# PranjalSahu/tensorflow_distributed

Hardware: AMD Instinct MI355X
Metric: images/sec (whole node) MNIST CNN DP at 1/2/4/8 MI355X; step-time scaling (higher is better)
Workload: dtype bf16; 1 GPU; global_batch=128, per_gpu_batch=128, parallelism=dp1, grad_allreduce=bf16, hipgraph=True, steps_per_graph=20, dp_transport=none, force_dp=False, zero1_fc1=False, fc_grads=bf16

## Files before the change

csrc/kernels/mnist.hip:

```cpp
#include "../common.h"

#include "../gemm.h"
#include "../gemm256.h"
#include "../launch_check.h"
#include "../mnist_layout.h"
#include "../tfd_kernels.h"
#include "../wt_store.h"
#include "../mnist_tail.h"

#include <algorithm>
#include <stdexcept>

constexpr int GEMM_RS = 2;
constexpr int FDX_BK_ = 128;
constexpr int FDW_BK_ = 64;
constexpr int FC1_BK_ = 32;

namespace tfd {
using namespace mnist;

namespace {

__device__ __forceinline__ int data_row(const int* perm, const int64_t* step, int n_data, int B, int b) {
  if (!perm) return b;
  const int64_t s = *step;
  return perm[(int)((s * (int64_t)B + b) % (int64_t)n_data)];
}
__device__ __forceinline__ int data_row(const MnistStepArgs& a, int b) {
  if (!a.perm) return b;
  if (a.rows) {
    const int tag = a.rows[a.B], r = a.rows[b];
    const int64_t s = *a.step;
    if (tag == (int)s) return r;
    return a.perm[(int)((s * (int64_t)a.B + b) % (int64_t)a.n_data)];
  }
  return data_row(a.perm, a.step, a.n_data, a.B, b);
}
struct RowPre {
  int64_t step;
  int tag, row;
};
__device__ __forceinline__ RowPre data_row_pre(const MnistStepArgs& a, int b) {
  RowPre r{0, -1, b};
  if (a.perm) {
    r.step = *a.step;
    if (a.rows) { r.tag = a.rows[a.B]; r.row = a.rows[b]; }
  }
  return r;
}
__device__ __forceinline__ int data_row_use(const MnistStepArgs& a, const RowPre& r, int b) {
  if (!a.perm) return b;
  if (a.rows && r.tag == (int)r.step) return r.row;
  return a.perm[(int)((r.step * (int64_t)a.B + b) % (int64_t)a.n_data)];
}
__device__ __forceinline__ int batch_label(const MnistStepArgs& a, int b) {
  if (a.perm && a.xpre) {
    const int tag = a.rows[a.B], y = a.ypre[b];
    const int64_t s = *a.step;
    if (tag == (int)s) return y;
  }
  return a.labels[data_row(a, b)];
}


constexpr int C2F_W = 24, C2F_PLANE = 18 * C2F_W, C2F_WLD = 48;
__device__ __forceinline__ int c2f_wrow(int r) { return (r >> 3) * 384 + (r & 7) * 32 + ((r >> 3) & 1) * 16; }
constexpr int C2F_WTAP = 4 * 384;
constexpr int C2F_WR4 = 4 * 32;
static_assert(C2F_WTAP == 32 * C2F_WLD, "the layout keeps the [800][48] footprint");
constexpr int C2L_FWD_SMEM = (4 * C2F_PLANE * 8 + 800 * C2F_WLD) * 2;
__device__ __forceinline__ void conv2_taps(const bf16* img, const bf16* wcol, const int base[2], f32x4 acc[2][2]) {
  bf16x8 a[2][2], b[2][2];
  auto load = [&](int tap, int slot) {
    const int kh = tap / 5, kw = tap - 5 * kh, toff = (kh * C2F_W + kw) * 8;
    const bf16* wr = wcol + tap * C2F_WTAP;
    b[slot][0] = frag_tr16(wr, wr + C2F_WR4);
    b[slot][1] = frag_tr16(wr + 16, wr + 16 + C2F_WR4);
    a[slot][0] = *reinterpret_cast<const bf16x8*>(img + base[0] + toff);
    a[slot][1] = *reinterpret_cast<const bf16x8*>(img + base[1] + toff);
  };
  load(0, 0);
#pragma unroll
  for (int tap = 0; tap < 25; ++tap) {
    const int cur = tap & 1;
    if (tap + 1 < 25) load(tap + 1, cur ^ 1);
#pragma unroll
    for (int j = 0; j < 2; ++j) {
      acc[j][0] = mfma16x16x32(a[cur][j], b[cur][0], acc[j][0]);
      acc[j][1] = mfma16x16x32(a[cur][j], b[cur][1], acc[j][1]);
    }
  }
}
static_assert(C2F_PLANE * 16 % 256 == 0, "chunk planes must be bank-row aligned");

constexpr int C12_XS = 36;
constexpr int C12_XR = 60;
constexpr int C12_XOFF = C2L_FWD_SMEM;
constexpr int C12_WOFF = C12_XOFF + C12_XR * C12_XS * 4;
constexpr int C12_IOFF = C12_WOFF + (KTAPS * C1 + C1) * 4;
constexpr int C12_X8P = 40;
constexpr int C12_X8OFF = C12_IOFF + 196 * 32;
constexpr int C12_SMEM = C12_X8OFF + 32 * C12_X8P * 16;
static_assert(C12_X8OFF % 16 == 0 && C12_SMEM <= 160 * 1024, "conv12 LDS carve");
static_assert(C12_IOFF % 16 == 0, "LDS carve alignment");
#ifndef TFD_STAMP
#define TFD_STAMP 0
#endif
#define C12_STAMP(k)                                                                       \
  do {                                                                                     \
    if (TFD_STAMP && a.dbg && threadIdx.x == 0) a.dbg[blockIdx.x * 16 + (k)] = (int64_t)__builtin_amdgcn_s_memtime(); \
  } while (0)
#define C12_STAMPW(k)                                                                      \
  do {                                                                                     \
    if (TFD_STAMP && a.dbg && threadIdx.x == 256) a.dbg[blockIdx.x * 16 + 8 + (k)] = (int64_t)__builtin_amdgcn_s_memtime(); \
  } while (0)
__global__ __launch_bounds__(512) void conv12_fwd_lds(MnistStepArgs a) {
  C12_STAMP(0);
  C12_STAMPW(0);
  extern __shared__ __attribute__((aligned(16))) char smem_raw[];
  bf16* img = (bf16*)smem_raw;
  bf16* wt = img + 4 * C2F_PLANE * 8;
  float* xs = reinterpret_cast<float*>(smem_raw + C12_XOFF);
  float* w1 = reinterpret_cast<float*>(smem_raw + C12_WOFF);
  const int b = blockIdx.x >> 1, nh = blockIdx.x & 1, t = threadIdx.x;
  const uint16_t* wsrc = a.pbf + OFF_WC2 + nh * 32;
  const int rot = (int)((blockIdx.x * 1031u) % 3200u);
  constexpr int NW = (3200 + 255) / 256;
  uint4 vw[NW];
#pragma unroll
  for (int j = 0; j < NW; ++j) vw[j] = zero4();
  f32x4 xv = f32x4{0.f, 0.f, 0.f, 0.f}, w1v = f32x4{0.f, 0.f, 0.f, 0.f};
  const int u = t - 256;
  const bool w2_role = __builtin_amdgcn_readfirstlane(t >> 6) < 4;
  if (w2_role) {
    const int tw = t & 255;
#pragma unroll
    for (int j = 0; j < NW; ++j) {
      const int e = tw + 256 * j, i = (min(e, 3199) + rot) % 3200;
      vw[j] = *reinterpret_cast<const uint4*>(wsrc + (i >> 2) * 64 + (i & 3) * 8);
    }
  } else {
    const int uw = min(u, (KTAPS * C1 + C1) / 4 - 1), ux = min(u, 195);
    w1v = reinterpret_cast<const f32x4*>(a.p32 + OFF_WC1)[uw];
    bool hit = false;
    if (a.perm && a.xpre) {
      xv = reinterpret_cast<const f32x4*>(a.xpre + (size_t)b * 784)[ux];
      hit = a.rows[a.B] == (int)*a.step;
    }
    if (!hit) {
      const float* x = a.data + (size_t)data_row(a, b) * 784;
      xv = reinterpret_cast<const f32x4*>(x)[ux];
    }
  }
  C12_STAMP(1);
  C12_STAMPW(1);
#if TFD_STAMP
  if (t == 256) {
    __builtin_amdgcn_s_waitcnt(0);
    C12_STAMPW(2);
  }
#endif
  for (int i = t; i < C12_XR * C12_XS / 4; i += 512) reinterpret_cast<f32x4*>(xs)[i] = f32x4{0.f, 0.f, 0.f, 0.f};
  for (int i = t; i < 4 * C2F_PLANE; i += 512) reinterpret_cast<uint4*>(img)[i] = zero4();
  C12_STAMPW(3);
  __syncthreads();
  C12_STAMPW(4);
  if (t >= 256) {
    if (u < (KTAPS * C1 + C1) / 4) reinterpret_cast<f32x4*>(w1)[u] = w1v;
    if (u < 196) {
      const int r = (4 * u) / 28, c = (4 * u) % 28;
      float* d = xs + (r + 2) * C12_XS + c + 2;
      d[0] = xv[0]; d[1] = xv[1]; d[2] = xv[2]; d[3] = xv[3];
    }
  }
  C12_STAMPW(5);
  __syncthreads();
  {
    bf16* x8 = reinterpret_cast<bf16*>(smem_raw + C12_X8OFF);
    for (int i = t; i < 32 * 28; i += 512) {
      const int r = i / 28, c = i - r * 28;
      const float* src = xs + r * C12_XS + c;
      bf16x8 e;
#pragma unroll
      for (int j = 0; j < 8; ++j) e[j] = (bf16)(j < 5 ? src[j] : 0.f);
      *reinterpret_cast<bf16x8*>(x8 + (r * C12_X8P + c) * 8) = e;
    }
    __syncthreads();
  }
  C12_STAMP(2);
  C12_STAMPW(6);
  {
    const int lane = t & 63, w = t >> 6, g = lane >> 4, col = lane & 15;
    uint8_t* idx_l = reinterpret_cast<uint8_t*>(smem_raw + C12_IOFF);
    const float bias0 = w1[KTAPS * C1 + col], bias1 = w1[KTAPS * C1 + 16 + col];
    constexpr int MT = 7;
    bf16x8 bw1[2], bw2[2];
#pragma unroll
    for (int nt = 0; nt < 2; ++nt)
#pragma unroll
      for (int jj = 0; jj < 8; ++jj) {
        const float r4 = jj < 5 ? w1[(20 + jj) * C1 + nt * 16 + col] : 0.f;
        bw1[nt][jj] = (bf16)(jj < 5 ? w1[(g * 5 + jj) * C1 + nt * 16 + col] : 0.f);
        bw2[nt][jj] = (bf16)(g == 0 ? r4 : 0.f);
      }
    const bf16* x8 = reinterpret_cast<const bf16*>(smem_raw + C12_X8OFF);
    bf16x8 af[MT], af2[MT];
#pragma unroll
    for (int i = 0; i < MT; ++i) {
      const int mt = w + 8 * i;
      const int m = min(mt, 48) * 16 + col, pp = m >> 2, win = m & 3;
      const int orow = 2 * (pp / 14) + (win >> 1), ocol = 2 * (pp % 14) + (win & 1);
      af[i] = *reinterpret_cast<const bf16x8*>(x8 + ((orow + g) * C12_X8P + ocol) * 8);
      af2[i] = *reinterpret_cast<const bf16x8*>(x8 + ((orow + 4) * C12_X8P + ocol) * 8);
    }
    f32x4 z[MT][2];
#pragma unroll
    for (int i = 0; i < MT; ++i)
#pragma unroll
      for (int nt = 0; nt < 2; ++nt)
        z[i][nt] = mfma16x16x32(af2[i], bw2[nt], mfma16x16x32(af[i], bw1[nt], f32x4{0.f, 0.f, 0.f, 0.f}));
#pragma unroll
    for (int i = 0; i < MT; ++i) {
      const int mt = w + 8 * i;
      if (mt >= 49) break;
      const int pq = mt * 4 + g, ph = pq / 14, pw = pq - ph * 14;
#pragma unroll
      for (int nt = 0; nt < 2; ++nt) {
        const int n = nt * 16 + col;
        const float bias = nt ? bias1 : bias0;
        float mx = z[i][nt][0] + bias;
        int am = 0;
#pragma unroll
        for (int r = 1; r < 4; ++r) {
          const float zz = z[i][nt][r] + bias;
          if (zz > mx) { mx = zz; am = r; }
        }
        reinterpret_cast<uint16_t*>(img)[((n >> 3) * C2F_PLANE + (ph + 2) * C2F_W + pw + 2) * 8 + (n & 7)] =
            f2bf_bits(fmaxf(mx, 0.f));
        idx_l[pq * 32 + n] = (uint8_t)am;
      }
    }
  }
  C12_STAMP(3);
  if (w2_role) {
#pragma unroll
    for (int j = 0; j < NW; ++j) {
      const int i = (t + 256 * j + rot) % 3200;
      if (t + 256 * j < 3200) *reinterpret_cast<uint4*>(wt + c2f_wrow(i >> 2) + (i & 3) * 8) = vw[j];
    }
  }
  __syncthreads();
  if (nh == 0) {
    const uint8_t* idx_l = reinterpret_cast<const uint8_t*>(smem_raw + C12_IOFF);
    const WtBuf bp1 = wt_buf(a.p1 + (size_t)b * 196 * 32, 196 * 32 * 2), bi1 = wt_buf(a.idx1 + (size_t)b * 196 * 32, 196 * 32);
    for (int i = t; i < 196 * 4; i += 512) {
      const int pq = i >> 2, cg = i & 3, ph = pq / 14, pw = pq - ph * 14;
      wt_store16(bp1, (uint32_t)i * 16u, true,
                 *reinterpret_cast<const uint4*>(img + (cg * C2F_PLANE + (ph + 2) * C2F_W + pw + 2) * 8));
    }
    for (int i = t; i < 196 * 2; i += 512) wt_store16(bi1, (uint32_t)i * 16u, true, reinterpret_cast<const uint4*>(idx_l)[i]);
  }
  C12_STAMP(4);
  const int lane = t & 63, w = t >> 6, g = lane >> 4, q = (lane & 15) >> 2, p4 = lane & 3;
  const int nmt = (w + 8 < 13) ? 2 : 1;
  int base[2];
  f32x4 acc[2][2];
#pragma unroll
  for (int j = 0; j < 2; ++j) {
    acc[j][0] = acc[j][1] = f32x4{0.f, 0.f, 0.f, 0.f};
    const int m = (w + 8 * j) * 16 + (lane & 15);
    int px = 0;
    if (m < 196) {
      const int pp = m >> 2, win = m & 3;
      px = (2 * (pp / 7) + (win >> 1)) * C2F_W + 2 * (pp % 7) + (win & 1);
    }
    base[j] = (g * C2F_PLANE + px) * 8;
  }
  const bf16* wcol = wt + c2f_wrow(8 * g + q) + 4 * p4;
  float bbv[2];
#pragma unroll
  for (int nt = 0; nt < 2; ++nt) bbv[nt] = a.p32[OFF_BC2 + nh * 32 + nt * 16 + (lane & 15)];
  conv2_taps(img, wcol, base, acc);
  C12_STAMP(5);
#pragma unroll
  for (int nt = 0; nt < 2; ++nt) {
    const int n = nh * 32 + nt * 16 + (lane & 15);
    const float bb = bbv[nt];
#pragma unroll
    for (int j = 0; j < 2; ++j) {
      const int m4 = (w + 8 * j) * 16 + 4 * g;
      if (j >= nmt || m4 >= 196) continue;
      float mx = acc[j][nt][0] + bb;
      int am = 0;
#pragma unroll
      for (int r = 1; r < 4; ++r) {
        const float z = acc[j][nt][r] + bb;
        if (z > mx) { mx = z; am = r; }
      }
      const size_t o = (size_t)b * FEAT + (m4 >> 2) * 64 + n;
      a.p2[o] = f2bf_bits(fmaxf(mx, 0.f));
      a.idx2[o] = (uint8_t)am;
    }
  }
  C12_STAMP(6);
}

struct SlabEpi {
  float* __restrict__ out;
  int ld, M, N;
  __device__ __forceinline__ void operator()(int m4, int n, f32x4 v) const {
    if (n >= N) return;
#pragma unroll
    for (int r = 0; r < 4; ++r)
      if (m4 + r < M) out[(size_t)(m4 + r) * ld + n] = v[r];
  }
};
constexpr int FC1_BM = 64, FC1_BN = 64, FC1_BK = FC1_BK_;
constexpr int FC1_SPLITS = 7;
constexpr int FC1_NKT = FEAT / FC1_SPLITS / FC1_BK;
static_assert(FC1_NKT * FC1_BK * FC1_SPLITS == FEAT, "fc1 split-K must tile K exactly");
__global__ __launch_bounds__(256) void fc1_fwd(MnistStepArgs a, int kper) {
  extern __shared__ __attribute__((aligned(16))) char smem_raw[];
  static_assert(FEAT % 8 == 0 && HID % 8 == 0, "whole chunks (DenseLoaderX)");
  DenseLoaderX<true> la{a.p2, FEAT, a.B, FEAT};
  DenseLoaderX<false> lb{a.pbf + OFF_WD1, HID, HID, FEAT};
  const int z = blockIdx.z;
  SlabEpi epi{a.fc1_slab + (size_t)z * a.B * HID, HID, a.B, HID};
  const int kb = z * kper;
  gemm_block_oneshot<FC1_BM, FC1_BN, FC1_BK, FC1_NKT, 2, 2>(la, lb, epi, blockIdx.y * FC1_BM, blockIdx.x * FC1_BN, kb, (bf16*)smem_raw);
}

#define HEAD_STAMP(k)                                                                                    \
  do {                                                                                                   \
    if (TFD_STAMP && a.dbg && threadIdx.x == 0) a.dbg[4 * a.B * 8 + blockIdx.x * 8 + (k)] = (int64_t)__builtin_amdgcn_s_memtime(); \
  } while (0)
__global__ __launch_bounds__(256) void head_kernel(MnistStepArgs a, int train) {
  HEAD_STAMP(0);
  const int row = blockIdx.x, t = threadIdx.x, lane = t & 63, wv = t >> 6;
  const int n0 = 4 * t;
  f32x4 p[FC1_SPLITS];
#pragma unroll
  for (int s = 0; s < FC1_SPLITS; ++s) p[s] = *reinterpret_cast<const f32x4*>(a.fc1_slab + ((size_t)s * a.B + row) * HID + n0);
  f32x4 wo[NCLS];
#pragma unroll
  for (int q = 0; q < NCLS; ++q) wo[q] = reinterpret_cast<const f32x4*>(a.p32 + OFF_OUT + (size_t)n0 * NCLS)[q];
#define HEAD_W(j, c) wo[((j) * NCLS + (c)) >> 2][((j) * NCLS + (c)) & 3]
  float bout[NCLS];
#pragma unroll
  for (int c = 0; c < NCLS; ++c) bout[c] = a.p32[OFF_BOUT + c];
  f32x4 h = *reinterpret_cast<const f32x4*>(a.p32 + OFF_BD1 + n0);
  const int64_t st = *a.step;
  const int lbl = batch_label(a, row);
  if (a.t_out && row == 0 && t == 0) *a.t_out = st + 1;
#pragma unroll
  for (int s = 0; s < FC1_SPLITS; ++s) h += p[s];
  HEAD_STAMP(1);
  float hd[4], scale[4];
  const float kp = train ? a.keep_prob : 1.0f;
  if (kp < 1.0f) {
    Philox4 r = philox4x32_10((uint32_t)(row * 256 + t), (uint32_t)st, (uint32_t)(st >> 32), a.rank, a.seed,
                              0x5EED1234u);
#pragma unroll
    for (int j = 0; j < 4; ++j) scale[j] = (u01(r.v[j]) < kp) ? (1.0f / kp) : 0.f;
  } else {
#pragma unroll
    for (int j = 0; j < 4; ++j) scale[j] = 1.f;
  }
#pragma unroll
  for (int j = 0; j < 4; ++j) hd[j] = fmaxf(h[j], 0.f) * scale[j];
  float lp[NCLS];
#pragma unroll
  for (int c = 0; c < NCLS; ++c) lp[c] = 0.f;
#pragma unroll
  for (int j = 0; j < 4; ++j) {
#pragma unroll
    for (int c = 0; c < NCLS; ++c) lp[c] = fmaf(hd[j], HEAD_W(j, c), lp[c]);
  }
  HEAD_STAMP(2);
  __shared__ float red[4][NCLS];
  wave_sums_to_lane63(lp);
  if (lane == 63) {
#pragma unroll
    for (int c = 0; c < NCLS; ++c) red[wv][c] = lp[c];
  }
  __syncthreads();
  float logit[NCLS];
#pragma unroll
  for (int c = 0; c < NCLS; ++c) logit[c] = red[0][c] + red[1][c] + red[2][c] + red[3][c] + bout[c];
  float mx = logit[0];
  int am = 0;
#pragma unroll
  for (int c = 1; c < NCLS; ++c)
    if (logit[c] > mx) { mx = logit[c]; am = c; }
  float se = 0.f;
#pragma unroll
  for (int c = 0; c < NCLS; ++c) se += __expf(logit[c] - mx);
  const float lse = mx + __logf(se);
  HEAD_STAMP(3);
  if (t == 0) {
    a.loss_row[row] = lse - logit[lbl];
    a.correct_row[row] = (am == lbl) ? 1.f : 0.f;
  }
  if (!train) return;
  const float invB = 1.0f / (float)a.B;
  float dl[NCLS];
#pragma unroll
  for (int c = 0; c < NCLS; ++c) dl[c] = (__expf(logit[c] - lse) - (c == lbl ? 1.f : 0.f)) * invB;
#pragma unroll
  for (int c = 0; c < NCLS; ++c)
    if (t == c) a.dlogits[row * NCLS + c] = dl[c];
  uint32_t hdw[2], dhw[2];
  float dhv[4];
#pragma unroll
  for (int j = 0; j < 4; ++j) {
    float d = 0.f;
#pragma unroll
    for (int c = 0; c < NCLS; ++c) d = fmaf(dl[c], HEAD_W(j, c), d);
    dhv[j] = (h[j] > 0.f) ? d * scale[j] : 0.f;
  }
#undef HEAD_W
  hdw[0] = pack_bf2(hd[0], hd[1]); hdw[1] = pack_bf2(hd[2], hd[3]);
  dhw[0] = pack_bf2(dhv[0], dhv[1]); dhw[1] = pack_bf2(dhv[2], dhv[3]);
  *reinterpret_cast<uint2*>(a.hd + (size_t)row * HID + n0) = make_uint2(hdw[0], hdw[1]);
  *reinterpret_cast<uint2*>(a.dh + (size_t)row * HID + n0) = make_uint2(dhw[0], dhw[1]);
  HEAD_STAMP(4);
}

constexpr int OUTG_ROWS = 64;
constexpr int LDS_PER_BLOCK = 160 * 1024;
constexpr int outg_smem(int B) { return (B * NCLS + 4 * OUTG_ROWS * NCLS) * 4; }
constexpr int OUTG_MAX_B = (LDS_PER_BLOCK / 4 - 4 * OUTG_ROWS * NCLS) / NCLS;
static_assert(outg_smem(OUTG_MAX_B) <= LDS_PER_BLOCK && outg_smem(OUTG_MAX_B + 1) > LDS_PER_BLOCK, "largest batch");
constexpr int OUTG_BLOCKS = (HID + 1 + OUTG_ROWS - 1) / OUTG_ROWS;
constexpr int OUTG_LB = 16;
__device__ __forceinline__ void out_grad_block(const MnistStepArgs& a, int blk, float* smem) {
  float* dl = smem;
  float* part = smem + a.B * NCLS;
  const int t = threadIdx.x, r = t & 63, q = t >> 6;
  for (int i = t; i < a.B * NCLS; i += 256) dl[i] = a.dlogits[i];
  __syncthreads();
  const int m = blk * OUTG_ROWS + r;
  float acc[NCLS];
#pragma unroll
  for (int c = 0; c < NCLS; ++c) acc[c] = 0.f;
  const int bq = (a.B + 3) >> 2, b0 = q * bq, b1 = min(a.B, b0 + bq);
  if (m < HID) {
    int b = b0;
    for (; b + OUTG_LB <= b1; b += OUTG_LB) {
      float hv[OUTG_LB];
#pragma unroll
      for (int u = 0; u < OUTG_LB; ++u) hv[u] = bf2f(a.hd[(size_t)(b + u) * HID + m]);
#pragma unroll
      for (int u = 0; u < OUTG_LB; ++u)
#pragma unroll
        for (int c = 0; c < NCLS; ++c) acc[c] = fmaf(hv[u], dl[(b + u) * NCLS + c], acc[c]);
    }
    for (; b < b1; ++b) {
      const float h = bf2f(a.hd[(size_t)b * HID + m]);
#pragma unroll
      for (int c = 0; c < NCLS; ++c) acc[c] = fmaf(h, dl[b * NCLS + c], acc[c]);
    }
  } else if (m == HID) {
    for (int b = b0; b < b1; ++b)
#pragma unroll
      for (int c = 0; c < NCLS; ++c) acc[c] += dl[b * NCLS + c];
  }
#pragma unroll
  for (int c = 0; c < NCLS; ++c) part[(q * 64 + r) * NCLS + c] = acc[c];
  __syncthreads();
  static_assert(OFF_OUT % 2 == 0 && NCLS % 2 == 0, "bf16 output-layer gradients are stored in pairs");
  auto gsum = [&](int i) {
    return part[i] + part[OUTG_ROWS * NCLS + i] + part[2 * OUTG_ROWS * NCLS + i] + part[3 * OUTG_ROWS * NCLS + i];
  };
  const int o0 = (int)OFF_OUT + blk * OUTG_ROWS * NCLS;
  if (a.gbf_a) {
    const WtBuf ob = wt_buf(a.gbf_a, TOTAL * 2);
    for (int i = 2 * t; i < OUTG_ROWS * NCLS; i += 512)
      wt_store4(ob, (uint32_t)(o0 + i) * 2u, blk * OUTG_ROWS + i / NCLS <= HID, pack_bf2(gsum(i), gsum(i + 1)));
  } else {
    const WtBuf ob = wt_buf(a.grad, TOTAL * 4);
    for (int i = t; i < OUTG_ROWS * NCLS; i += 256)
      wt_store4(ob, (uint32_t)(o0 + i) * 4u, blk * OUTG_ROWS + i / NCLS <= HID, __float_as_uint(gsum(i)));
  }
}

struct OnesRowBuf {
  static constexpr bool KC = false;
  const uint16_t* __restrict__ x;
  int k_lim;
  uint32_t nbytes;
  __device__ __forceinline__ uint4 operator()(int mn, int k) const {
    const uint4 v = buf_ld(x, nbytes, (uint32_t)k * FEAT + mn, k < k_lim && mn < FEAT);
    return (mn == FEAT && k < k_lim) ? make_uint4(0x3F80u, 0u, 0u, 0u) : v;
  }
};
static_assert(FEAT % 8 == 0, "the ones row starts a fresh 8-element chunk");

constexpr int FDW_BM = 64, FDW_BN = 64, FDW_BK = FDW_BK_;
constexpr int FDW_PITCH = FDW_BN + 4;
__device__ __forceinline__ void fc1_dw_store(f32x4 (&acc)[2][2], float* cs, float* out, uint16_t* outbf, int m0,
                                             int n0, int M) {
  const int tid = threadIdx.x, lane = tid & 63, w = tid >> 6, wm = w >> 1, wn = w & 1;
#pragma unroll
  for (int i = 0; i < 2; ++i)
#pragma unroll
    for (int j = 0; j < 2; ++j)
#pragma unroll
      for (int r = 0; r < 4; ++r)
        cs[(wm * 32 + 16 * i + 4 * (lane >> 4) + r) * FDW_PITCH + wn * 32 + 16 * j + (lane & 15)] = acc[i][j][r];
  __syncthreads();
#pragma unroll
  for (int q = tid; q < FDW_BM * FDW_BN / 8; q += 256) {
    const int row = q >> 3, ch = q & 7, m = m0 + row;
    const f32x4 lo = *reinterpret_cast<const f32x4*>(cs + row * FDW_PITCH + ch * 8);
    const f32x4 hi = *reinterpret_cast<const f32x4*>(cs + row * FDW_PITCH + ch * 8 + 4);
    const uint32_t o = (uint32_t)(m * HID + n0 + ch * 8);
    if (outbf) {
      wt_store16(wt_buf(outbf, (int64_t)M * HID * 2), o * 2u, m < M,
                 make_uint4(pack_bf2(lo[0], lo[1]), pack_bf2(lo[2], lo[3]), pack_bf2(hi[0], hi[1]), pack_bf2(hi[2], hi[3])));
    } else {
      const WtBuf ob = wt_buf(out, (int64_t)M * HID * 4);
      wt_store16(ob, o * 4u, m < M, f4_bits(lo));
      wt_store16(ob, o * 4u + 16u, m < M, f4_bits(hi));
    }
  }
}
template <class LA, class LB>
__device__ __forceinline__ void fc1_dw_tile(const MnistStepArgs& a, const LA& la, const LB& lb, int m0, int n0, int K,
                                            bf16* smem) {
  f32x4 acc[2][2];
  gemm_mainloop<FDW_BM, FDW_BN, FDW_BK, 2, 2, LA, LB, GEMM_RS>(la, lb, m0, n0, 0, K, smem, acc);
  fc1_dw_store(acc, reinterpret_cast<float*>(smem), a.grad + OFF_WD1, a.gbf_a ? a.gbf_a + OFF_WD1 : nullptr, m0, n0,
               FEAT + 1);
}
__device__ __forceinline__ void fc1_dw_block(const MnistStepArgs& a, int bx, int by, bf16* smem) {
  OnesRowBuf la{a.p2, a.B, (uint32_t)((int64_t)a.B * FEAT * 2)};
  DenseLoaderX<false> lb{a.dh, HID, HID, a.B};
  fc1_dw_tile(a, la, lb, by * FDW_BM, bx * FDW_BN, a.B, smem);
}

constexpr int FDX_BM = 32, FDX_BN = 64, FDX_BK = FDX_BK_, FDX_BN2 = 32;
template <int BN>
__device__ __forceinline__ void fc1_dx_unpool_store(const MnistStepArgs& a, f32x4 (&acc)[FDX_BM / 32][BN / 32],
                                                    float* cs, int m0, int n0) {
  constexpr int PITCH = BN + 4, CPR = BN / 8;
  const int tid = threadIdx.x, lane = tid & 63, w = tid >> 6, wm = w >> 1, wn = w & 1;
  constexpr int WTM = FDX_BM / 2, WTN = BN / 2;
  const int b = tid / CPR, cc = tid % CPR, m = m0 + b;
  const bool live = b < FDX_BM && m < a.B;
  const size_t xo = (size_t)(live ? m : 0) * FEAT + n0 + cc * 8;
  const uint4 pv = *reinterpret_cast<const uint4*>(a.p2 + xo);
  const uint2 iv = *reinterpret_cast<const uint2*>(a.idx2 + xo);
#pragma unroll
  for (int i = 0; i < WTM / 16; ++i)
#pragma unroll
    for (int j = 0; j < WTN / 16; ++j)
#pragma unroll
      for (int r = 0; r < 4; ++r)
        cs[(wm * WTM + 16 * i + 4 * (lane >> 4) + r) * PITCH + wn * WTN + 16 * j + (lane & 15)] = acc[i][j][r];
  __syncthreads();
  if (!live) return;
  const f32x4 lo = *reinterpret_cast<const f32x4*>(cs + b * PITCH + cc * 8);
  const f32x4 hi = *reinterpret_cast<const f32x4*>(cs + b * PITCH + cc * 8 + 4);
// ... 716 lines not shown
```

Baseline: 2.253 million images/s.

## Build conv1 im2col and bf16 weight fragments directly in LDS, split output stores

The fused conv1/conv2 forward kernel no longer stages the input image and conv1 weights as fp32 in LDS before converting them. Input rows are packed straight into the bf16 shifted-window layout with alignbit, and conv1 weights are pre-packed into bf16x8 MFMA fragments. Only the padding borders are zeroed instead of whole planes. This removes one block barrier and a conversion pass. The pool1/index global stores are now split across both block halves instead of done by nh==0 alone. The cost is more intricate indexing logic that must exactly reproduce the previous padding.

```diff
diff --git a/csrc/kernels/mnist.hip b/csrc/kernels/mnist.hip
--- a/csrc/kernels/mnist.hip
+++ b/csrc/kernels/mnist.hip
@@ -93,16 +93,15 @@
 }
 static_assert(C2F_PLANE * 16 % 256 == 0, "chunk planes must be bank-row aligned");
 
-constexpr int C12_XS = 36;
-constexpr int C12_XR = 60;
-constexpr int C12_XOFF = C2L_FWD_SMEM;
-constexpr int C12_WOFF = C12_XOFF + C12_XR * C12_XS * 4;
-constexpr int C12_IOFF = C12_WOFF + (KTAPS * C1 + C1) * 4;
+constexpr int C12_WFN = 2 * 4 * 16 + 2 * 16;
+constexpr int C12_WOFF = C2L_FWD_SMEM;
+constexpr int C12_IOFF = C12_WOFF + C12_WFN * 16;
 constexpr int C12_X8P = 40;
 constexpr int C12_X8OFF = C12_IOFF + 196 * 32;
 constexpr int C12_SMEM = C12_X8OFF + 32 * C12_X8P * 16;
-static_assert(C12_X8OFF % 16 == 0 && C12_SMEM <= 160 * 1024, "conv12 LDS carve");
+static_assert(C12_X8OFF % 16 == 0 && C12_SMEM <= 143424, "conv12 LDS carve");
 static_assert(C12_IOFF % 16 == 0, "LDS carve alignment");
+typedef uint32_t u32x4 __attribute__((ext_vector_type(4)));
 #ifndef TFD_STAMP
 #define TFD_STAMP 0
 #endif
@@ -120,8 +119,6 @@
   extern __shared__ __attribute__((aligned(16))) char smem_raw[];
   bf16* img = (bf16*)smem_raw;
   bf16* wt = img + 4 * C2F_PLANE * 8;
-  float* xs = reinterpret_cast<float*>(smem_raw + C12_XOFF);
-  float* w1 = reinterpret_cast<float*>(smem_raw + C12_WOFF);
   const int b = blockIdx.x >> 1, nh = blockIdx.x & 1, t = threadIdx.x;
   const uint16_t* wsrc = a.pbf + OFF_WC2 + nh * 32;
   const int rot = (int)((blockIdx.x * 1031u) % 3200u);
@@ -129,80 +126,111 @@
   uint4 vw[NW];
 #pragma unroll
   for (int j = 0; j < NW; ++j) vw[j] = zero4();
-  f32x4 xv = f32x4{0.f, 0.f, 0.f, 0.f}, w1v = f32x4{0.f, 0.f, 0.f, 0.f};
-  const int u = t - 256;
-  const bool w2_role = __builtin_amdgcn_readfirstlane(t >> 6) < 4;
-  if (w2_role) {
-    const int tw = t & 255;
+  const int tw = t & 255;
+  auto load_w2 = [&]() {
 #pragma unroll
     for (int j = 0; j < NW; ++j) {
       const int e = tw + 256 * j, i = (min(e, 3199) + rot) % 3200;
       vw[j] = *reinterpret_cast<const uint4*>(wsrc + (i >> 2) * 64 + (i & 3) * 8);
     }
+  };
+  auto zero_borders = [&]() {
+    const int pl = t >> 7, e = t & 127;
+    int r, c;
+    if (e < 72) {
+      const int rr = e / 18;
+      r = rr + (rr >= 2 ? 14 : 0);
+      c = e - rr * 18;
+    } else {
+      const int f = e - 72, cc = f & 3;
+      r = 2 + (f >> 2);
+      c = cc + (cc >= 2 ? 14 : 0);
+    }
+    reinterpret_cast<uint4*>(img)[pl * C2F_PLANE + r * C2F_W + c] = zero4();
+    if (t < 4 * 28) {
+      const int rr = t / 28;
+      reinterpret_cast<uint4*>(smem_raw + C12_X8OFF)[(rr + (rr >= 2 ? 28 : 0)) * C12_X8P + t - rr * 28] = zero4();
+    }
+  };
+  float bias0, bias1;
+  if (__builtin_amdgcn_readfirstlane(t >> 6) < 4) {
+    bias0 = a.p32[OFF_BC1 + (t & 15)];
+    bias1 = a.p32[OFF_BC1 + 16 + (t & 15)];
+    load_w2();
+    C12_STAMP(1);
+    zero_borders();
   } else {
-    const int uw = min(u, (KTAPS * C1 + C1) / 4 - 1), ux = min(u, 195);
-    w1v = reinterpret_cast<const f32x4*>(a.p32 + OFF_WC1)[uw];
+    const int u = t - 256, e = min(u, C12_WFN - 1);
+    const int tap0 = e < 128 ? ((e >> 4) & 3) * 5 : 20, ch = e < 128 ? (e >> 6) * 16 + (e & 15) : e - 128;
+    float w1t[5];
+    bias0 = a.p32[OFF_BC1 + (t & 15)];
+    bias1 = a.p32[OFF_BC1 + 16 + (t & 15)];
+#pragma unroll
+    for (int jj = 0; jj < 5; ++jj) w1t[jj] = a.p32[OFF_WC1 + (tap0 + jj) * C1 + ch];
+    const int ux = min(u, 195), un = min(u + 1, 195);
+    f32x4 xv = f32x4{0.f, 0.f, 0.f, 0.f}, xn = f32x4{0.f, 0.f, 0.f, 0.f};
     bool hit = false;
     if (a.perm && a.xpre) {
-      xv = reinterpret_cast<const f32x4*>(a.xpre + (size_t)b * 784)[ux];
+      const f32x4* x = reinterpret_cast<const f32x4*>(a.xpre + (size_t)b * 784);
+      xv = x[ux];
+      xn = x[un];
       hit = a.rows[a.B] == (int)*a.step;
     }
     if (!hit) {
-      const float* x = a.data + (size_t)data_row(a, b) * 784;
-      xv = reinterpret_cast<const f32x4*>(x)[ux];
-    }
-  }
-  C12_STAMP(1);
-  C12_STAMPW(1);
+      const f32x4* x = reinterpret_cast<const f32x4*>(a.data + (size_t)data_row(a, b) * 784);
+      xv = x[ux];
+      xn = x[un];
+    }
+    C12_STAMPW(1);
 #if TFD_STAMP
-  if (t == 256) {
-    __builtin_amdgcn_s_waitcnt(0);
-    C12_STAMPW(2);
-  }
+    if (t == 256) {
+      __builtin_amdgcn_s_waitcnt(0);
+      C12_STAMPW(2);
+    }
 #endif
-  for (int i = t; i < C12_XR * C12_XS / 4; i += 512) reinterpret_cast<f32x4*>(xs)[i] = f32x4{0.f, 0.f, 0.f, 0.f};
-  for (int i = t; i < 4 * C2F_PLANE; i += 512) reinterpret_cast<uint4*>(img)[i] = zero4();
-  C12_STAMPW(3);
-  __syncthreads();
-  C12_STAMPW(4);
-  if (t >= 256) {
-    if (u < (KTAPS * C1 + C1) / 4) reinterpret_cast<f32x4*>(w1)[u] = w1v;
+    zero_borders();
+    C12_STAMPW(3);
+    if (u < C12_WFN)
+      reinterpret_cast<u32x4*>(smem_raw + C12_WOFF)[u] =
+          u32x4{pack_bf2(w1t[0], w1t[1]), pack_bf2(w1t[2], w1t[3]), (uint32_t)f2bf_bits(w1t[4]), 0u};
     if (u < 196) {
-      const int r = (4 * u) / 28, c = (4 * u) % 28;
-      float* d = xs + (r + 2) * C12_XS + c + 2;
-      d[0] = xv[0]; d[1] = xv[1]; d[2] = xv[2]; d[3] = xv[3];
-    }
+      const int r = u / 7, k7 = u - 7 * r;
+      const bool last = k7 == 6;
+      const uint32_t d0 = pack_bf2(xv[0], xv[1]), d1 = pack_bf2(xv[2], xv[3]);
+      const uint32_t d2 = last ? 0u : pack_bf2(xn[0], xn[1]), d3 = last ? 0u : pack_bf2(xn[2], xn[3]);
+      const uint32_t s01 = __builtin_amdgcn_alignbit(d1, d0, 16), s12 = __builtin_amdgcn_alignbit(d2, d1, 16),
+                     s23 = __builtin_amdgcn_alignbit(d3, d2, 16);
+      u32x4* row = reinterpret_cast<u32x4*>(smem_raw + C12_X8OFF) + (r + 2) * C12_X8P;
+      const int c0 = 4 * k7 + 2;
+      row[c0] = u32x4{d0, d1, d2 & 0xFFFFu, 0u};
+      row[c0 + 1] = u32x4{s01, s12, d2 >> 16, 0u};
+      if (!last) {
+        row[c0 + 2] = u32x4{d1, d2, d3 & 0xFFFFu, 0u};
+        row[c0 + 3] = u32x4{s12, s23, d3 >> 16, 0u};
+      }
+      if (k7 == 0) {
+        row[0] = u32x4{0u, d0, d1 & 0xFFFFu, 0u};
+        row[1] = u32x4{d0 << 16, s01, d1 >> 16, 0u};
+      }
+    }
+    C12_STAMPW(4);
   }
   C12_STAMPW(5);
   __syncthreads();
-  {
-    bf16* x8 = reinterpret_cast<bf16*>(smem_raw + C12_X8OFF);
-    for (int i = t; i < 32 * 28; i += 512) {
-      const int r = i / 28, c = i - r * 28;
-      const float* src = xs + r * C12_XS + c;
-      bf16x8 e;
-#pragma unroll
-      for (int j = 0; j < 8; ++j) e[j] = (bf16)(j < 5 ? src[j] : 0.f);
-      *reinterpret_cast<bf16x8*>(x8 + (r * C12_X8P + c) * 8) = e;
-    }
-    __syncthreads();
-  }
   C12_STAMP(2);
   C12_STAMPW(6);
   {
     const int lane = t & 63, w = t >> 6, g = lane >> 4, col = lane & 15;
     uint8_t* idx_l = reinterpret_cast<uint8_t*>(smem_raw + C12_IOFF);
-    const float bias0 = w1[KTAPS * C1 + col], bias1 = w1[KTAPS * C1 + 16 + col];
     constexpr int MT = 7;
+    const u32x4* wf = reinterpret_cast<const u32x4*>(smem_raw + C12_WOFF);
     bf16x8 bw1[2], bw2[2];
 #pragma unroll
-    for (int nt = 0; nt < 2; ++nt)
-#pragma unroll
-      for (int jj = 0; jj < 8; ++jj) {
-        const float r4 = jj < 5 ? w1[(20 + jj) * C1 + nt * 16 + col] : 0.f;
-        bw1[nt][jj] = (bf16)(jj < 5 ? w1[(g * 5 + jj) * C1 + nt * 16 + col] : 0.f);
-        bw2[nt][jj] = (bf16)(g == 0 ? r4 : 0.f);
-      }
+    for (int nt = 0; nt < 2; ++nt) {
+      const u32x4 r4 = wf[128 + nt * 16 + col];
+      bw1[nt] = __builtin_bit_cast(bf16x8, wf[nt * 64 + g * 16 + col]);
+      bw2[nt] = __builtin_bit_cast(bf16x8, g == 0 ? r4 : u32x4{0u, 0u, 0u, 0u});
+    }
     const bf16* x8 = reinterpret_cast<const bf16*>(smem_raw + C12_X8OFF);
     bf16x8 af[MT], af2[MT];
 #pragma unroll
@@ -219,6 +247,7 @@
 #pragma unroll
       for (int nt = 0; nt < 2; ++nt)
         z[i][nt] = mfma16x16x32(af2[i], bw2[nt], mfma16x16x32(af[i], bw1[nt], f32x4{0.f, 0.f, 0.f, 0.f}));
+    C12_STAMP(7);
 #pragma unroll
     for (int i = 0; i < MT; ++i) {
       const int mt = w + 8 * i;
@@ -242,7 +271,7 @@
     }
   }
   C12_STAMP(3);
-  if (w2_role) {
+  if (t < 256) {
 #pragma unroll
     for (int j = 0; j < NW; ++j) {
       const int i = (t + 256 * j + rot) % 3200;
@@ -250,15 +279,18 @@
     }
   }
   __syncthreads();
-  if (nh == 0) {
+  {
     const uint8_t* idx_l = reinterpret_cast<const uint8_t*>(smem_raw + C12_IOFF);
     const WtBuf bp1 = wt_buf(a.p1 + (size_t)b * 196 * 32, 196 * 32 * 2), bi1 = wt_buf(a.idx1 + (size_t)b * 196 * 32, 196 * 32);
-    for (int i = t; i < 196 * 4; i += 512) {
-      const int pq = i >> 2, cg = i & 3, ph = pq / 14, pw = pq - ph * 14;
+    if (t < 196 * 2) {
+      const int i = nh * 196 * 2 + t, pq = i >> 2, cg = i & 3, ph = pq / 14, pw = pq - ph * 14;
       wt_store16(bp1, (uint32_t)i * 16u, true,
                  *reinterpret_cast<const uint4*>(img + (cg * C2F_PLANE + (ph + 2) * C2F_W + pw + 2) * 8));
     }
-    for (int i = t; i < 196 * 2; i += 512) wt_store16(bi1, (uint32_t)i * 16u, true, reinterpret_cast<const uint4*>(idx_l)[i]);
+    if (t < 196) {
+      const int i = nh * 196 + t;
+      wt_store16(bi1, (uint32_t)i * 16u, true, reinterpret_cast<const uint4*>(idx_l)[i]);
+    }
   }
   C12_STAMP(4);
   const int lane = t & 63, w = t >> 6, g = lane >> 4, q = (lane & 15) >> 2, p4 = lane & 3;
```

Result: no change. 2.260 million images/s, median of 6 (+0.3%).
